# uw-math-ai/TheoremSearch

Hardware: AMD Instinct MI355X
Metric: queries/sec, brute-force top-10 over N x 768 theorem embeddings (higher is better)
Workload: dtype bf16; 1 GPU; 10000000x768 bf16 corpus, batch-256 queries, top-10 (BASELINE.json configs[2]); rows=10000000, dim=768, batch=256, k=10, searches_in_flight=1, parallelism=corpus row-sharded x1

## Files before the change

theoremsearch_amd/csrc/kernels_mfma16.h:

```cpp
#pragma once
#include <type_traits>

#include "kernels_mfma16_ops.h"
#include "kernels_screen8_tile.h"
#include "mfma16_variants.h"

namespace ts {

constexpr int kMfma16PrivCap = 16;
constexpr int kMfma16StageCap = 192;
constexpr int kMfma16StageBytes = 4 * kMfma16StageCap * 16 + 16;
constexpr int kMfma16PaceBytes = 256;

__device__ __forceinline__ u64 mfma16_block_test(const f32x4& a0, const f32x4& a1, float thr, float& m) {
    u64 mask;
    asm volatile(
        "v_max3_f32 %0, %2, %3, %4\n\t"
        "v_max3_f32 %0, %0, %5, %6\n\t"
        "v_max3_f32 %0, %0, %7, %8\n\t"
        "v_max_f32 %0, %0, %9\n\t"
        "v_cmp_ge_f32 %1, %0, %10"
        : "=&v"(m), "=s"(mask)
        : "v"(a0[0]), "v"(a0[1]), "v"(a0[2]), "v"(a0[3]), "v"(a1[0]), "v"(a1[1]), "v"(a1[2]), "v"(a1[3]), "v"(thr));
    return mask;
// ... 146 lines not shown
    constexpr int kUnits = dims::kUnits, kUnitBytes = dims::kUnitBytes, kSlots = dims::kSlots, kPieces = dims::kPieces;
    constexpr int kUnitK = dims::kUnitK;
    constexpr int kPieceEvery = kUnitSteps / kPieces;
    static_assert(kUnitSteps % kPieces == 0 && kPieceEvery >= 1, "DMA pieces must spread evenly over the k-steps");
    static_assert(!KSPLIT || (kUnitSteps == 4 && kPieces == 4), "k-split: four k-steps and four DMA pieces per unit and wave");
    static_assert(NB >= 1 && NB * kSteps * 4 <= 384, "query fragments must fit the register file");
    static_assert(!F32 || NB <= 2, "the fp32 issue order is written for one or two query blocks per wave");
    static_assert(kUnits == 1 || kUnits == 2 || kUnits == 4 || kUnits == 8, "units per tile");
    constexpr bool kStaged = !SPARSE;
    constexpr int kFrags = NB * kSteps;
    constexpr int kA = (kUnitSteps % 3 == 0) ? 3 : 4;
    constexpr int kQVmax = (KSPLIT || kLate) ? 24 : 36 - 2 * (kA - 2);
    constexpr int kQV = kFrags < kQVmax ? kFrags : kQVmax;
    constexpr bool kStreamNT = !PAIR;
    extern __shared__ __attribute__((aligned(16))) unsigned char smem[];
    const int lane = threadIdx.x & 63;
    const int wave = __builtin_amdgcn_readfirstlane(threadIdx.x >> 6);
    const int r16 = lane & 15, kq = lane >> 4;
    const int wg = PAIR ? (int)(((blockIdx.x >> 4) << 3) | (blockIdx.x & 7)) : (int)blockIdx.x;
    const int qhalf = PAIR ? (int)((blockIdx.x >> 3) & 1) : 0;
    const int G = PAIR ? (int)(gridDim.x >> 1) : (int)gridDim.x;
    const int nwriters = 4 * gridDim.x;
    const int writer = 4 * blockIdx.x + kq;
    const int khalf = KSPLIT ? (wave >> 1) : 0;
    int qid[NB];
#pragma unroll
    for (int b = 0; b < NB; ++b)
        qid[b] = KSPLIT ? qhalf * 128 + (((b + 2 * khalf) & 3) * 2 + (wave & 1)) * 16 + r16 : qhalf * 64 * NB + (b * 4 + wave) * 16 + r16;

    mfma_level_begin(a);
    uint4* stage = (uint4*)(smem + dims::kLds) + wave * kMfma16StageCap;
    uint2* stage8 = (uint2*)(smem + dims::kLds) + wave * kScreenStageCap;
    static_assert(kScreenStageCap * 8 == kMfma16StageCap * 16, "the screen's entries fill the same LDS");
    u32* stage_cnt = (u32*)(smem + dims::kLds + 4 * kMfma16StageCap * 16) + wave;
    if (kStaged && !I8 && lane == 0) *stage_cnt = 0;
    uint4* const xbuf = (uint4*)(smem + dims::kLds + kMfma16StageBytes + kMfma16PaceBytes);
    frag16 got[4] = {};
    const bool pace = PAIR && a.pair_pos != nullptr && a.pair_lag > 0 && wave == 0;
    unsigned* const pace_mine = PAIR ? a.pair_pos + 2 * wg + qhalf : nullptr;
    const unsigned* const pace_partner = PAIR ? a.pair_pos + 2 * wg + (1 - qhalf) : nullptr;
    unsigned pace_seen = 0, pace_prev = 0, pace_v;
    if (PAIR && wave == 0) ((u32*)(smem + dims::kLds + kMfma16StageBytes))[lane] = 0;
    const unsigned long long wg_start = (!SPARSE && a.wg_ticks) ? __builtin_amdgcn_s_memrealtime() : 0ull;
    const int64_t t0 = (!SPARSE && a.part) ? a.part[wg] : (a.ntiles * (int64_t)wg) / G;
    const int nt = (int)(((!SPARSE && a.part) ? a.part[wg + 1] : (a.ntiles * (int64_t)(wg + 1)) / G) - t0);
    if (nt <= 0) {
        if (!SPARSE && a.wg_ticks && threadIdx.x == 0 && qhalf == 0) a.wg_ticks[wg] = 0;
        if (!kStaged) {
#pragma unroll
            for (int b = 0; b < NB; ++b) a.pcount[(int64_t)qid[b] * nwriters + writer] = 0;
        }
        return;
    }
    const int nu = kUnits * nt;
    const int drow = 8 * wave + (lane >> 3);
    const int dchunk = (lane & 7) ^ ((drow >> 1) & 7);
    const int64_t tile_bytes = (int64_t)kTileRows * Deq * 2;
    const int64_t run_jump = tile_bytes * ((int64_t)a.run * a.tile_stride - a.run + 1);
    const int64_t g0 = (t0 / a.run) * a.run * a.tile_stride + t0 % a.run;
    const unsigned char* tile_src = (const unsigned char*)a.corpus + (int64_t)drow * (Deq * 2) + dchunk * 16 + g0 * tile_bytes;
    int issue_run_pos = (int)(t0 % a.run);
    int issue_u = 0, issue_ui = 0, issue_slot = 0;
    const unsigned lds_base = (unsigned)(unsigned long long)(__attribute__((address_space(3))) unsigned char*)smem;
    const unsigned lds0 = lds_base + wave * 1024;
    const unsigned pace_word = __builtin_amdgcn_readfirstlane(lds_base + dims::kLds + kMfma16StageBytes);
    const unsigned xfetch = lds_base + dims::kLds + kMfma16StageBytes + kMfma16PaceBytes + (((wave ^ 2) * 256 + lane) << 4);

    const int lane_off = (r16 >> 3) * 1024 + (r16 & 7) * 128;
    const int sw = (r16 >> 1) & 7;
    int xo[2];
#pragma unroll
    for (int sp = 0; sp < 2; ++sp) xo[sp] = lane_off + (((4 * sp + kq) ^ sw) << 4);
    const unsigned koff = KSPLIT ? (unsigned)(khalf * (kUnitSteps / 2) * 4096) : 0u;

#define TS16_ISSUED()                                                                 \
    do {                                                                              \
        if (++issue_ui == kUnits) {                                                   \
            issue_ui = 0;                                                             \
            tile_src += (issue_run_pos + 1 == a.run) ? run_jump : tile_bytes;         \
            issue_run_pos = (issue_run_pos + 1 == a.run) ? 0 : issue_run_pos + 1;     \
        }                                                                             \
        ++issue_u;                                                                    \
        issue_slot = (issue_slot + 1 == kSlots) ? 0 : issue_slot + 1;                 \
    } while (0)

    const int ahead = (a.ahead >= 2 && a.ahead < kSlots) ? a.ahead : kSlots - 1;
    for (int i = 0; i < ahead && issue_u < nu && !kNoDma; ++i) {
        const unsigned char* src = tile_src + issue_ui * (kUnitK * 2);
#pragma unroll
        for (int j = 0; j < kPieces; ++j) lds_dma16<kStreamNT>(src + j * 128, lds0 + issue_slot * kUnitBytes + j * 4096);
        TS16_ISSUED();
    }
    bf16x8 qv[kQV], qa[kFrags > kQV ? kFrags - kQV : 1];
#pragma unroll
    for (int b = 0; b < NB; ++b) {
        const bf16x8* pq = F32 ? (const bf16x8*)((const float*)a.q + (int64_t)qid[b] * D + 4 * kq)
                               : (const bf16x8*)(a.q + (int64_t)qid[b] * D + 8 * kq);
        if (KSPLIT) pq += 4 * kUnitSteps * khalf;
#pragma unroll
        for (int ks = 0; ks < kSteps; ++ks) {
            const int f = b * kSteps + ks;
            const int kabs = KSPLIT ? (ks / kUnitSteps) * kUnitStepsAll + (ks % kUnitSteps) : ks;
            if (f < kQV) qv[f < kQV ? f : 0] = pq[4 * kabs];
            else qa[f >= kQV ? f - kQV : 0] = pq[4 * kabs];
        }
    }
    float thr[NB];
#pragma unroll
    for (int b = 0; b < NB; ++b) thr[b] = mfma_level_thr(a, qid[b]);
    float fq1[I8 ? NB : 1], fq2[I8 ? NB : 1], fq3[I8 ? NB : 1];
    if constexpr (I8) {
#pragma unroll
        for (int b = 0; b < NB; ++b) {
            const float4 m4 = a.scr_q[qid[b]];
            screen_fold_query(thr[b], m4.x, m4.y, m4.z, fq1[b], fq2[b], fq3[b]);
        }
    }
#pragma unroll
    for (int f = 0; f < kFrags; ++f) {
        if (f < kQV) asm volatile("" : "+v"(qv[f < kQV ? f : 0]));
        else asm volatile("" : "+a"(qa[f >= kQV ? f - kQV : 0]));
    }
#pragma unroll
    for (int b = 0; b < NB; ++b) asm volatile("" : "+v"(thr[b]));
    if constexpr (I8) {
#pragma unroll
        for (int b = 0; b < NB; ++b) asm volatile("" : "+v"(fq1[b]), "+v"(fq2[b]), "+v"(fq3[b]));
    }

    asm volatile("s_waitcnt vmcnt(0)" ::: "memory");
    __builtin_amdgcn_s_barrier();
    asm volatile("" ::: "memory");

    frag16 af[2 * kA] = {};
    {
        const unsigned p0 = lds_base + xo[0] + (KSPLIT ? khalf * (kUnitSteps / 2) * 4096 : 0);
        const unsigned p1 = lds_base + xo[1] + (KSPLIT ? khalf * (kUnitSteps / 2) * 4096 : 0);
        lds_read16<0>(af[0], p0);
        lds_read16<2048>(af[1], p0);
        lds_read16<0>(af[2], p1);
        lds_read16<2048>(af[3], p1);
        if constexpr (kA > 3) {
            lds_read16<4096>(af[4], p0);
            lds_read16<4096 + 2048>(af[5], p0);
        }
        static_assert(kA == 3 || kA == 4, "prologue written for rings of 3 or 4 k-steps");
    }
    lds_ring_landed(af);

    f32x4 acc[2][NB];
    f32x4 accK[2][2][2] = {};
    f32x4 accL[kLate ? 2 : 1][2][kLate ? NB : 1];
    int lthr[kLate ? 2 : 1][kLate ? NB : 1];
    int lbest = 0;
    u64 lhit[kLate ? NB : 1];
    u64 lany = 0, lany2 = 0;
    if constexpr (kLate) {
#pragma unroll
        for (int b = 0; b < NB; ++b) {
            accL[1][0][b] = f32x4{0.0f, 0.0f, 0.0f, 0.0f};
            accL[1][1][b] = f32x4{0.0f, 0.0f, 0.0f, 0.0f};
            lthr[1][b] = 0x7fffffff;
            asm volatile("" : "+v"(accL[1][0][b]), "+v"(accL[1][1][b]), "+v"(lthr[1][b]));
        }
    }
    u32 cnt[NB];
#pragma unroll
    for (int b = 0; b < NB; ++b) cnt[b] = 0;
    int slot = 0, u = 0;
    unsigned long long t_vm = 0, t_bar = 0, t_dma = 0, t_all0 = 0;
    unsigned long long t_tail = 0;
    if (kStamps) t_all0 = cycle_stamp();
    unsigned long long c_begin = 0, r_begin = 0;
    if (kProbe) {
        c_begin = __builtin_amdgcn_s_memtime();
        r_begin = __builtin_amdgcn_s_memrealtime();
        __builtin_amdgcn_s_waitcnt(0xC07F);
    }

#define TS16_ACC(RB_, B_) (*((KSPLIT && (B_) < 2) ? &accK[par_][RB_][(B_) & 1] : &acc[RB_][B_]))
#define TS16_MMA(RB_, B_, KS_, AF_)                                                                        \
    do {                                                                                                   \
        constexpr int f_ = (B_) * kSteps + (KS_);                                                          \
        if constexpr (kLate) {                                                                             \
            if constexpr ((KS_) == 0 && f_ < kQV) mfma8_v_first(accL[par_][RB_][B_], AF_, qv[f_ < kQV ? f_ : 0]);  \
            else if constexpr ((KS_) == 0) mfma8_a_first(accL[par_][RB_][B_], AF_, qa[f_ >= kQV ? f_ - kQV : 0]); \
            else if constexpr (f_ < kQV) mfma8_v(accL[par_][RB_][B_], AF_, qv[f_ < kQV ? f_ : 0]);         \
            else mfma8_a(accL[par_][RB_][B_], AF_, qa[f_ >= kQV ? f_ - kQV : 0]);                          \
        } else if constexpr (I8) {                                                                         \
            if constexpr ((KS_) == 0 && f_ < kQV) mfma8_v_first(acc[RB_][B_], AF_, qv[f_ < kQV ? f_ : 0]);  \
            else if constexpr ((KS_) == 0) mfma8_a_first(acc[RB_][B_], AF_, qa[f_ >= kQV ? f_ - kQV : 0]); \
            else if constexpr (f_ < kQV) mfma8_v(acc[RB_][B_], AF_, qv[f_ < kQV ? f_ : 0]);                \
            else mfma8_a(acc[RB_][B_], AF_, qa[f_ >= kQV ? f_ - kQV : 0]);                                 \
        } else if constexpr ((KS_) == 0) {                                                                 \
            if constexpr (f_ < kQV) mfma16_v_first(TS16_ACC(RB_, B_), AF_, qv[f_ < kQV ? f_ : 0]);         \
            else mfma16_a_first(TS16_ACC(RB_, B_), AF_, qa[f_ >= kQV ? f_ - kQV : 0]);                     \
        } else {                                                                                           \
            if constexpr (f_ < kQV) mfma16_v(TS16_ACC(RB_, B_), AF_, qv[f_ < kQV ? f_ : 0]);               \
            else mfma16_a(TS16_ACC(RB_, B_), AF_, qa[f_ >= kQV ? f_ - kQV : 0]);                           \
        }                                                                                                  \
    } while (0)
#define TS16_MMAF(RB_, B_, KS_, AF_, I_)                                                                   \
    do {                                                                                                   \
        constexpr int f_ = (B_) * kSteps + (KS_);                                                          \
        const f32x4& af4_ = reinterpret_cast<const f32x4&>(AF_);                                           \
        if constexpr ((KS_) == 0 && (I_) == 0) {                                                           \
            if constexpr (f_ < kQV) mfma16f_v_first(acc[RB_][B_], af4_[I_], reinterpret_cast<const f32x4&>(qv[f_ < kQV ? f_ : 0])[I_]); \
            else mfma16f_a_first(acc[RB_][B_], af4_[I_], reinterpret_cast<const f32x4&>(qa[f_ >= kQV ? f_ - kQV : 0])[I_]); \
        } else if constexpr (f_ < kQV) {                                                                   \
            mfma16f_v(acc[RB_][B_], af4_[I_], reinterpret_cast<const f32x4&>(qv[f_ < kQV ? f_ : 0])[I_]);  \
        } else {                                                                                           \
            mfma16f_a(acc[RB_][B_], af4_[I_], reinterpret_cast<const f32x4&>(qa[f_ >= kQV ? f_ - kQV : 0])[I_]); \
        }                                                                                                  \
    } while (0)

#define TS16_LOAD(RB_, N_)                                                                                 \
    do {                                                                                                   \
        constexpr int w_ = 2 * ((N_) % kA) + (RB_);                                                        \
        if constexpr ((N_) < kUnitSteps) lds_read16<((N_) >> 1) * 4096 + (RB_) * 2048>(af[w_], ua[(N_) & 1]); \
        else lds_read16<(((N_) - kUnitSteps) >> 1) * 4096 + (RB_) * 2048>(af[w_], na[(N_) & 1]);          \
    } while (0)
#define TS16_PIECE(S_)                                                                                     \
    do {                                                                                                   \
        if constexpr ((S_) % kPieceEvery == kPieceEvery - 1)                                               \
            if (do_issue) {                                                                                \
                constexpr int j_ = (S_) / kPieceEvery;                                                     \
                unsigned long long d0_ = 0;                                                                \
                if (VARIANT == kVariantStamps) d0_ = cycle_stamp();                                        \
                if constexpr (steady_) lds_dma16s<j_ * 128, kStreamNT>(dma_voff, ssrc, idst + j_ * (4096 - 128 * TS16_DMA_IMM_LDS)); \
                else lds_dma16<kStreamNT>(isrc + j_ * 128, idst + j_ * 4096);                                         \
                if (VARIANT == kVariantStamps) t_dma += cycle_stamp() - d0_;                               \
            }                                                                                              \
    } while (0)
#define TS16_FILL(KS_, G_)                                                                                 \
    do {                                                                                                   \
        constexpr int fi_ = ((KS_) - (kSteps - 3)) * 4 + (G_);                                             \
        if constexpr (KSPLIT && !kNoEpi && (KS_) >= kSteps - 3) {                                          \
            if constexpr (fi_ == 0) {                                                                      \
                asm volatile("" : "+v"(got[0]), "+v"(got[1]), "+v"(got[2]), "+v"(got[3]));                 \
                ksplit_add4(sum_[0][0], accK[par_ ^ 1][0][0], reinterpret_cast<const f32x4&>(got[0]));               \
            }                                                                                              \
            if constexpr (fi_ == 1) ksplit_add4(sum_[1][0], accK[par_ ^ 1][1][0], reinterpret_cast<const f32x4&>(got[2])); \
            if constexpr (fi_ == 2) ksplit_add4(sum_[0][1], accK[par_ ^ 1][0][1], reinterpret_cast<const f32x4&>(got[1])); \
            if constexpr (fi_ == 3) ksplit_add4(sum_[1][1], accK[par_ ^ 1][1][1], reinterpret_cast<const f32x4&>(got[3])); \
            if constexpr (fi_ == 4) ksplit_test_a(best_[0], sum_[0][0], sum_[1][0]);                       \
            if constexpr (fi_ == 5) ksplit_test_b(best_[0], sum_[1][0]);                                   \
            if constexpr (fi_ == 6) ksplit_test_c(hit_[0], best_[0], thr[0]);                              \
            if constexpr (fi_ == 7) ksplit_test_a(best_[1], sum_[0][1], sum_[1][1]);                       \
            if constexpr (fi_ == 8) ksplit_test_b(best_[1], sum_[1][1]);                                   \
            if constexpr (fi_ == 9) ksplit_test_c(hit_[1], best_[1], thr[1]);                              \
        }                                                                                                  \
    } while (0)
#define TS16_THR8(KS_, G_)                                                                                 \
    do {                                                                                                   \
        if constexpr (I8 && !kNoEpi) {                                                                     \
            constexpr int gpk_ = NB >= 3 ? 4 : 2;                                                          \
            constexpr int g_ = NB == 1 ? (G_) + 2 : (G_);                                                  \
            constexpr int P_ = ((KS_) / 2) * gpk_ + g_;                                                    \
            if constexpr ((KS_) % 2 == 0 && g_ >= 0 && g_ < gpk_ && (NB == 1) == ((G_) < 0) && P_ < 4 * NB) { \
                if constexpr (kLate) screen_thr_piece<P_ & 3>(lthr[par_][P_ >> 2], tml[par_], fq1[P_ >> 2], fq2[P_ >> 2], fq3[P_ >> 2]); \
                else screen_thr_piece<P_ & 3>(ithr[P_ >> 2], tmc, fq1[P_ >> 2], fq2[P_ >> 2], fq3[P_ >> 2]);   \
            }                                                                                              \
        }                                                                                                  \
    } while (0)
#define TS16_LATE(KS_, G_)                                                                                 \
    do {                                                                                                   \
        if constexpr (kLate) {                                                                             \
            constexpr int p_ = (KS_) * 2 + (G_);                                                           \
            if constexpr (p_ < 3 * NB) {                                                                   \
                constexpr int b_ = p_ / 3;                                                                 \
                if constexpr (p_ % 3 == 0) late_test_a(lbest, accL[par_ ^ 1][0][b_], accL[par_ ^ 1][1][b_]); \
                if constexpr (p_ % 3 == 1) late_test_b(lbest, accL[par_ ^ 1][1][b_]);                      \
                if constexpr (p_ % 3 == 2) late_test_c(lhit[b_], lbest, lthr[par_ ^ 1][b_]);               \
            }                                                                                              \
            if constexpr (p_ == 3 * NB) late_or(lany, lhit[0], lhit[1]);                                   \
            if constexpr (p_ == 3 * NB + 1) late_or(lany2, lhit[2], lhit[3]);                              \
            if constexpr (p_ == 3 * NB + 2) late_or(lany, lany, lany2);                                    \
            if constexpr (steady_ && p_ == 2 * (kSteps - kA)) {    \
                asm volatile("" : "+s"(noff_l));                   \
                la_l[0] = lds_base + noff_l + xo[0] + koff;                                                \
                la_l[1] = lds_base + noff_l + xo[1] + koff;                                                \
                asm volatile("" : "+v"(la_l[0]), "+v"(la_l[1]));                                           \
                na[0] = la_l[0]; na[1] = la_l[1];                                                          \
            }                                                                                              \
            if constexpr (steady_ && p_ == 2 * kSteps - 2) {                                               \
                poff = soff;                                                                               \
                soff = noff_l;                                                                             \
                noff_l = (soff + kUnitBytes == (unsigned)dims::kLds) ? 0u : soff + kUnitBytes;             \
                s_tile += steady_jump;                                                                     \
                asm volatile("" : "+s"(poff), "+s"(soff), "+s"(noff_l), "+s"(s_tile));                     \
            }                                                                                              \
            if constexpr (steady_ && p_ == 2 * kSteps - 1) {                                               \
                sp_l += 1;                                                                                 \
                asm volatile("" : "+s"(sp_l));                                                             \
            }                                                                                              \
        }                                                                                                  \
    } while (0)
#ifndef TS16_ORDER_A
#define TS16_BF16_ORDER(KS_, R0_, N_, S_)                                                                  \
    do {                                                                                                   \
        if constexpr (KSPLIT) {                                                                            \
            TS16_MMA(0, 2, KS_, af[R0_]); TS16_LOAD(0, N_);                                                \
            TS16_MMA(1, 2, KS_, af[R0_ + 1]); TS16_LOAD(1, N_);                                            \
            TS16_MMA(0, 3, KS_, af[R0_]); TS16_MMA(1, 3, KS_, af[R0_ + 1]);                                \
            TS16_PIECE(S_);                                                                                \
            TS16_MMA(0, 0, KS_, af[R0_]); TS16_FILL(KS_, 0);                                               \
            TS16_MMA(1, 0, KS_, af[R0_ + 1]); TS16_FILL(KS_, 1);                                           \
            TS16_MMA(0, 1, KS_, af[R0_]); TS16_FILL(KS_, 2);                                               \
            TS16_MMA(1, 1, KS_, af[R0_ + 1]); TS16_FILL(KS_, 3);                                           \
            break;                                                                                         \
        }                                                                                                  \
        TS16_MMA(0, 0, KS_, af[R0_]); TS16_LOAD(0, N_); TS16_THR8(KS_, -2);                                \
        TS16_MMA(1, 0, KS_, af[R0_ + 1]); TS16_LOAD(1, N_); TS16_THR8(KS_, -1);                            \
        if constexpr (NB > 1) {                                                                            \
            TS16_MMA(0, 1, KS_, af[R0_]); TS16_THR8(KS_, 0);                                               \
            TS16_MMA(1, 1, KS_, af[R0_ + 1]); TS16_THR8(KS_, 1);                                           \
        }                                                                                                  \
        TS16_PIECE(S_);                                                                                    \
        if constexpr (NB > 2) {                                                                            \
            TS16_MMA(0, 2, KS_, af[R0_]); TS16_THR8(KS_, 2);                                               \
            TS16_MMA(1, 2, KS_, af[R0_ + 1]); TS16_THR8(KS_, 3);                                           \
        }                                                                                                  \
        if constexpr (NB > 3) { TS16_MMA(0, 3, KS_, af[R0_]); TS16_LATE(KS_, 0); TS16_MMA(1, 3, KS_, af[R0_ + 1]); TS16_LATE(KS_, 1); } \
    } while (0)
#else
#define TS16_BF16_ORDER(KS_, R0_, N_, S_)                                                                  \
    do {                                                                                                   \
        TS16_MMA(0, 0, KS_, af[R0_]); TS16_LOAD(0, N_);                                                    \
        if constexpr (NB > 1) { TS16_MMA(0, 1, KS_, af[R0_]); }                                            \
        TS16_LOAD(1, N_);                                                                                  \
        if constexpr (NB > 2) { TS16_MMA(0, 2, KS_, af[R0_]); }                                            \
        if constexpr (NB > 3) { TS16_MMA(0, 3, KS_, af[R0_]); }                                            \
        TS16_PIECE(S_);                                                                                    \
        TS16_MMA(1, 0, KS_, af[R0_ + 1]);                                                                  \
        if constexpr (NB > 1) { TS16_MMA(1, 1, KS_, af[R0_ + 1]); }                                        \
        if constexpr (NB > 2) { TS16_MMA(1, 2, KS_, af[R0_ + 1]); }                                        \
        if constexpr (NB > 3) { TS16_MMA(1, 3, KS_, af[R0_ + 1]); }                                        \
    } while (0)
#endif
#define TS16_STEP(UI, S_)                                                                                  \
    do {                                                                                                   \
        constexpr int ks_ = (UI) * kUnitSteps + (S_);                                                      \
        constexpr int r0_ = 2 * ((S_) % kA);                                                               \
        constexpr int n_ = (S_) + kA - 1;                                                                  \
        if constexpr (!kNoMma) {                                                                           \
             \
                         \
            if constexpr (kA == 3) asm volatile("s_waitcnt lgkmcnt(2)" : "+v"(af[r0_]), "+v"(af[r0_ + 1])); \
            else asm volatile("s_waitcnt lgkmcnt(4)" : "+v"(af[r0_]), "+v"(af[r0_ + 1]));                  \
        }                                                                                                  \
        if constexpr (!kNoMma && F32) {                                                                    \
                           \
            TS16_MMAF(0, 0, ks_, af[r0_], 0); TS16_LOAD(0, n_);                                            \
            TS16_MMAF(1, 0, ks_, af[r0_ + 1], 0); TS16_LOAD(1, n_);                                        \
            if constexpr (NB > 1) { TS16_MMAF(0, 1, ks_, af[r0_], 0); TS16_MMAF(1, 1, ks_, af[r0_ + 1], 0); } \
            TS16_MMAF(0, 0, ks_, af[r0_], 1); TS16_MMAF(1, 0, ks_, af[r0_ + 1], 1);                        \
            TS16_PIECE(S_);                                                                                \
            if constexpr (NB > 1) { TS16_MMAF(0, 1, ks_, af[r0_], 1); TS16_MMAF(1, 1, ks_, af[r0_ + 1], 1); } \
            TS16_MMAF(0, 0, ks_, af[r0_], 2); TS16_MMAF(1, 0, ks_, af[r0_ + 1], 2);                        \
            if constexpr (NB > 1) { TS16_MMAF(0, 1, ks_, af[r0_], 2); TS16_MMAF(1, 1, ks_, af[r0_ + 1], 2); } \
            TS16_MMAF(0, 0, ks_, af[r0_], 3); TS16_MMAF(1, 0, ks_, af[r0_ + 1], 3);                        \
            if constexpr (NB > 1) { TS16_MMAF(0, 1, ks_, af[r0_], 3); TS16_MMAF(1, 1, ks_, af[r0_ + 1], 3); } \
        }                                                                                                  \
        if constexpr (!kNoMma && !F32) {                                                                   \
             \
            TS16_BF16_ORDER(ks_, r0_, n_, S_);                                                             \
        }                                                                                                  \
        if constexpr (kNoMma) TS16_PIECE(S_);                                                              \
    } while (0)

#define TS16_KSPLIT_FETCH()                                                                                \
    do {                                                                                                   \
        lds_read16<0>(got[0], xfetch); lds_read16<1024>(got[1], xfetch);                                   \
        lds_read16<2048>(got[2], xfetch); lds_read16<3072>(got[3], xfetch);                                \
    } while (0)
#define TS16_UNIT_S(UI)                                                                                    \
    do {                                                                                                   \
        constexpr int cui_ = ((UI) + kSlots - 1) % kUnits;                                                 \
         \
        const unsigned noff = kLate ? noff_l : (soff + kUnitBytes == (unsigned)dims::kLds) ? 0u : soff + kUnitBytes; \
        unsigned ua[2], na[2];                                                                             \
        if constexpr (!kLate) {                                                                            \
            ua[0] = lds_base + soff + xo[0] + koff; ua[1] = lds_base + soff + xo[1] + koff;                \
            na[0] = lds_base + noff + xo[0] + koff; na[1] = lds_base + noff + xo[1] + koff;                \
        } else {    \
            ua[0] = la_l[0]; ua[1] = la_l[1];                                                              \
        }                                                                                                  \
        if constexpr (!kNoDma) wait_vmcnt<(kSlots - 3) * kPieces>();          \
        if constexpr (PAIR && (UI) == (2 % kUnits)) {                    \
             \
                            \
            asm volatile("v_readfirstlane_b32 %0, %1" : "=s"(pace_seen) : "v"(pace_v));                   \
            const int ahead_ = (int)((unsigned)t - pace_seen);                                             \
            if (pace && pace_seen != pace_prev && ahead_ > a.pair_lag && ahead_ < (1 << 20))               \
                for (int z_ = 0; z_ < ahead_ - a.pair_lag && z_ < 4; ++z_) __builtin_amdgcn_s_sleep(5);    \
            pace_prev = pace_seen;                                                                         \
        }                                                                                                  \
        __builtin_amdgcn_s_barrier();                                               \
        asm volatile("" ::: "memory");                                                                     \
        if constexpr (KSPLIT && (UI) == 2) TS16_KSPLIT_FETCH();                                            \
        if constexpr (PAIR && (UI) == 0) {                                                                 \
            if (pace) pair_publish_and_fetch(pace_mine, pace_partner, (unsigned)t, pace_word);            \
        }                                                                                                  \
        if constexpr (PAIR && (UI) == (1 % kUnits)) pair_read_word(pace_v, pace_word);                     \
        if (VARIANT == kVariantSleep) __builtin_amdgcn_s_sleep(4);                                         \
        constexpr bool do_issue = !kNoDma;                                                                 \
        constexpr bool steady_ = true;                                                                     \
        const unsigned char* isrc = nullptr;                                                               \
        const unsigned char* ssrc = s_tile + cui_ * (kUnitK * 2);                  \
        const unsigned idst = lds0 + poff;                                                                 \
        TS16_STEP(UI, 0); TS16_STEP(UI, 1); TS16_STEP(UI, 2); TS16_STEP(UI, 3);                            \
        if constexpr (kUnitSteps > 4) { TS16_STEP(UI, 4 % kUnitSteps); TS16_STEP(UI, 5 % kUnitSteps); TS16_STEP(UI, 6 % kUnitSteps); TS16_STEP(UI, 7 % kUnitSteps); } \
        if constexpr (kUnitSteps > 8) { TS16_STEP(UI, 8 % kUnitSteps); TS16_STEP(UI, 9 % kUnitSteps); TS16_STEP(UI, 10 % kUnitSteps); TS16_STEP(UI, 11 % kUnitSteps); } \
        if constexpr (!kLate) {                                                                            \
            if constexpr (cui_ == kUnits - 1 && !kNoDma) s_tile += steady_jump;                            \
            poff = soff;                                                                                   \
            soff = noff;                                                                                   \
        }                                                                                                  \
    } while (0)

#define TS16_UNIT(UI)                                                                                      \
    do {                                                                                                   \
        const int nslot = (slot + 1 == kSlots) ? 0 : slot + 1;                                             \
        unsigned ua[2], na[2];                                                                             \
        ua[0] = lds_base + slot * kUnitBytes + xo[0] + koff; ua[1] = lds_base + slot * kUnitBytes + xo[1] + koff;   \
        na[0] = lds_base + nslot * kUnitBytes + xo[0] + koff; na[1] = lds_base + nslot * kUnitBytes + xo[1] + koff; \
         \
        unsigned long long s0_ = 0, s1_ = 0;                                                               \
        if (kStamps) s0_ = cycle_stamp();                                                                  \
        if (u + 1 < nu && !kNoDma) wait_keep_units<kPieces>(issue_u - (u + 2));                            \
        if (kStamps) s1_ = cycle_stamp();                                                                  \
        __builtin_amdgcn_s_barrier();                                                                      \
        asm volatile("" ::: "memory");                                                                     \
        if constexpr (KSPLIT && (UI) == 2) TS16_KSPLIT_FETCH();                                            \
        if (kStamps) { t_vm += s1_ - s0_; t_bar += cycle_stamp() - s1_; }                                  \
        if (VARIANT == kVariantSleep) __builtin_amdgcn_s_sleep(4);    \
        const bool do_issue = issue_u < nu && !kNoDma;                                                     \
        constexpr bool steady_ = false;                                                                    \
        const unsigned char* isrc = tile_src + issue_ui * (kUnitK * 2);                                    \
        const unsigned char* ssrc = nullptr;                                                               \
         \
        const unsigned idst = __builtin_amdgcn_readfirstlane(lds0 + issue_slot * kUnitBytes);              \
        TS16_STEP(UI, 0); TS16_STEP(UI, 1); TS16_STEP(UI, 2); TS16_STEP(UI, 3);                            \
        if constexpr (kUnitSteps > 4) { TS16_STEP(UI, 4 % kUnitSteps); TS16_STEP(UI, 5 % kUnitSteps); TS16_STEP(UI, 6 % kUnitSteps); TS16_STEP(UI, 7 % kUnitSteps); } \
        if constexpr (kUnitSteps > 8) { TS16_STEP(UI, 8 % kUnitSteps); TS16_STEP(UI, 9 % kUnitSteps); TS16_STEP(UI, 10 % kUnitSteps); TS16_STEP(UI, 11 % kUnitSteps); } \
        if (do_issue) TS16_ISSUED();                                                                       \
        slot = nslot;                                                                                      \
        ++u;                                                                                               \
    } while (0)

#define TS16_KSPLIT_APPEND(TP)                                                                             \
    do {                                                                                                   \
        if (__builtin_expect((hit_[0] | hit_[1]) != 0, 0)) {                                               \
            const int64_t lt_ = t0 + (TP);                                                                 \
            const int64_t tile_row_ = (a.run == 1 ? lt_ * a.tile_stride : (lt_ / a.run) * a.run * a.tile_stride + lt_ % a.run) * kTileRows; \
            const int64_t row_base_ = tile_row_ + 4 * kq;                                                  \
            _Pragma("unroll") for (int i_ = 0; i_ < 2; ++i_)                                               \
                if (hit_[i_] != 0)                                                                         \
                    mfma16_append_block<kStaged>(sum_[0][i_], sum_[1][i_], thr[i_], best_[i_], qid[i_], writer, nwriters, cnt[i_], \
                                                 row_base_, a, stage, stage_cnt);                          \
        }                                                                                                  \
    } while (0)
    static_assert(kUnitSteps == 8 || kUnitSteps == 12 || (KSPLIT && kUnitSteps == 4), "unit = 8 or 12 k-steps of 32 (k-split: this wave's 4 of 8)");
    static_assert(kSlots >= 3, "the steady part keeps kSlots - 3 units in flight behind its wait");
    const int nt_steady = (a.run == 1 && ahead == kSlots - 1 && !kStamps && nu > ahead) ? (nu - ahead) / kUnits : 0;
    const int64_t steady_jump = tile_bytes * a.tile_stride;
    unsigned soff = 0, poff = (unsigned)(kSlots - 1) * kUnitBytes;
    unsigned noff_l = (unsigned)kUnitBytes;
    unsigned la_l[2] = {lds_base + xo[0] + koff, lds_base + xo[1] + koff};
    static_assert(!kLate || kUnits == 1, "the late-test screen advances the stream's tile base once per unit");
    const unsigned dma_voff = (unsigned)(drow * (Deq * 2) + dchunk * 16);
    const unsigned char* s_tile = (const unsigned char*)a.corpus + (t0 + ahead / kUnits) * steady_jump;
    f32x4 sum_[2][2] = {};
    float best_[2] = {};
    u64 hit_[2] = {};
    const tile_scalars_ptr scr_tile = (tile_scalars_ptr)a.scr_tile;
    f32x4 tmc = {0.0f, 0.0f, 0.0f, 0.0f}, tmn = {0.0f, 0.0f, 0.0f, 0.0f};
    f32x4 tml[2] = {{0.0f, 0.0f, 0.0f, 0.0f}, {0.0f, 0.0f, 0.0f, 0.0f}};
    tile_scalars_ptr sp_l = scr_tile + (t0 + 1);
    int ithr[I8 ? NB : 1];
    u32 scnt = 0, s_n = 0, s_nq = 0;
    int t_chk = 0;
    screen_u32_gptr s_count = nullptr;
    screen_u64_gptr s_cand = nullptr;
    screen_mask_cptr s_mask = nullptr;
    if constexpr (I8) {
        if constexpr (kLate) {
            screen_tile_scalars(tml[0], scr_tile, t0);
            screen_tile_scalars(tml[1], scr_tile, t0 + (nt > 1 ? 1 : 0));
            asm volatile("" : "+s"(tml[0]), "+s"(tml[1]), "+s"(sp_l));
        } else {
            screen_tile_scalars(tmc, scr_tile, t0);
            screen_tile_scalars(tmn, scr_tile, t0 + (nt > 1 ? 1 : 0));
            asm volatile("" : "+s"(tmc), "+s"(tmn));
        }
        const int64_t whole = a.n / kTileRows - t0;
        t_chk = whole < (int64_t)nt ? (whole > 0 ? (int)whole : 0) : nt;
        s_n = (u32)a.n;
        s_nq = (u32)a.nq_real;
        s_count = (screen_u32_gptr)a.count;
        s_cand = (screen_u64_gptr)a.cand;
        asm volatile("" : "+s"(scnt), "+s"(t_chk), "+s"(s_n), "+s"(s_nq), "+s"(s_count), "+s"(s_cand));
        if constexpr (kMasked8) {
            s_mask = (screen_mask_cptr)a.row_mask;
            asm volatile("" : "+s"(s_mask));
        }
    }
    constexpr int kTilePick = 0, kTileSteady = 1, kTileGeneral = 2;
    auto tile = [&](auto par_c, auto form_c, const int t) __attribute__((always_inline)) {
        constexpr int par_ = decltype(par_c)::value;
        constexpr int form_ = decltype(form_c)::value;
        (void)par_;
        unsigned long long tail0 = 0;
        if (form_ == kTileSteady || (form_ == kTilePick && t < nt_steady)) {
            TS16_UNIT_S(0);
            if constexpr (kUnits >= 2) TS16_UNIT_S(1 % kUnits);
            if constexpr (kUnits >= 4) {
                TS16_UNIT_S(2 % kUnits);
                TS16_UNIT_S(3 % kUnits);
            }
            if constexpr (kUnits == 8) {
                TS16_UNIT_S(4 % kUnits);
                TS16_UNIT_S(5 % kUnits);
                TS16_UNIT_S(6 % kUnits);
                TS16_UNIT_S(7 % kUnits);
            }
            if constexpr (!kNoMma) lds_ring_landed(af);
            if (form_ == kTilePick && t + 1 == nt_steady) {
                u = kUnits * nt_steady;
                slot = u % kSlots;
                issue_u = u + ahead;
                issue_ui = issue_u % kUnits;
                issue_slot = issue_u % kSlots;
                issue_run_pos = 0;
                tile_src = s_tile + dma_voff;
            }
        } else {
            TS16_UNIT(0);
            if constexpr (kUnits >= 2) TS16_UNIT(1 % kUnits);
            if constexpr (kUnits >= 4) {
                TS16_UNIT(2 % kUnits);
                TS16_UNIT(3 % kUnits);
            }
            if constexpr (kUnits == 8) {
                TS16_UNIT(4 % kUnits);
                TS16_UNIT(5 % kUnits);
                TS16_UNIT(6 % kUnits);
                TS16_UNIT(7 % kUnits);
            }
            if (VARIANT == kVariantScreenStamps) tail0 = cycle_stamp();
            if constexpr (!kNoMma) lds_ring_landed(af);
        }
        if constexpr (kNoMma) return;
        if constexpr (KSPLIT) {
            if constexpr (kNoEpi) {
                asm volatile("s_nop 15\n\ts_nop 3" : "+v"(accK[par_][0][0]), "+v"(accK[par_][0][1]), "+v"(accK[par_][1][0]), "+v"(accK[par_][1][1]),
                             "+v"(acc[0][2]), "+v"(acc[0][3]), "+v"(acc[1][2]), "+v"(acc[1][3]));
                return;
            }
            if (t > 0) TS16_KSPLIT_APPEND(t - 1);
            ksplit_hand_over(acc, xbuf + wave * 256 + lane);
            return;
        }
#ifdef TS16_ORDER_A
        mfma16_settle<NB>(acc);
#else
        if constexpr (NB < 4 || kNoEpi) mfma16_settle<NB>(acc);
#endif
        if constexpr (kNoEpi) {
#pragma unroll
            for (int b = 0; b < NB; ++b) asm volatile("" ::"v"(acc[0][b]), "v"(acc[1][b]));
            return;
        }
        if constexpr (kLate) {
            asm volatile("" : "+s"(tml[par_ ^ 1]));
            if constexpr (form_ == kTileSteady) tml[par_] = *(const volatile __attribute__((address_space(4))) f32x4*)sp_l;
            if (__builtin_expect(lany != 0, 0)) {
                const u32 tp = (u32)t0 + (u32)t - 1u;
                const u32 row_base = tp * kTileRows + 4 * kq;
                if (t - 1 >= t_chk) {
                    const u32 live = screen_tile_live<false>(tp * kTileRows, s_n, s_mask) >> (4 * kq);
#pragma unroll
                    for (int b = 0; b < NB; ++b)
                        if (lhit[b] != 0)
                            mfma8_append_block<true>(accL[par_ ^ 1][0][b], accL[par_ ^ 1][1][b], lthr[par_ ^ 1][b], qid[b], row_base, scnt, stage8, live, s_nq, s_count, s_cand);
                } else {
#pragma unroll
                    for (int b = 0; b < NB; ++b)
                        if (lhit[b] != 0)
                            mfma8_append_block<false>(accL[par_ ^ 1][0][b], accL[par_ ^ 1][1][b], lthr[par_ ^ 1][b], qid[b], row_base, scnt, stage8, 0u, s_nq, s_count, s_cand);
                }
            }
            if constexpr (form_ != kTileSteady) screen_tile_scalars(tml[par_], scr_tile, t0 + (t + 2 < nt ? t + 2 : nt - 1));
            return;
        }
        if constexpr (I8) {
            asm volatile("" : "+s"(tmn));
            u64 ihit[NB];
            const u64 iany = screen_tile_test<NB>(acc, ithr, ihit);
            if constexpr (variant_test_only(VARIANT)) {
                asm volatile("" ::"s"(iany));
            } else if (__builtin_expect(iany != 0, 0)) {
                const u32 row_base = ((u32)t0 + (u32)t) * kTileRows + 4 * kq;
                if (kMasked8 || t >= t_chk) {
                    const u32 live = screen_tile_live<kMasked8>(((u32)t0 + (u32)t) * kTileRows, s_n, s_mask) >> (4 * kq);
#pragma unroll
                    for (int b = 0; b < NB; ++b)
                        if (ihit[b] != 0)
                            mfma8_append_block<true>(acc[0][b], acc[1][b], ithr[b], qid[b], row_base, scnt, stage8, live, s_nq, s_count, s_cand);
                } else {
#pragma unroll
                    for (int b = 0; b < NB; ++b)
                        if (ihit[b] != 0)
                            mfma8_append_block<false>(acc[0][b], acc[1][b], ithr[b], qid[b], row_base, scnt, stage8, 0u, s_nq, s_count, s_cand);
                }
            }
            if (VARIANT == kVariantScreenStamps) t_tail += cycle_stamp() - tail0;
            tmc = tmn;
            screen_tile_scalars(tmn, scr_tile, t0 + (t + 2 < nt ? t + 2 : nt - 1));
            return;
        }
        mfma16_tile_tail<NB, VARIANT, kStaged>(acc, thr, qid, cnt, t0, t, kq, writer, nwriters, a, stage, stage_cnt);
    };
    using tile_pick = std::integral_constant<int, kTilePick>;
    if constexpr (kLate) {
        int t = 0;
        const int t_trips = __builtin_amdgcn_readfirstlane(nt_steady & ~1);
        if (t_trips > 0) {
            do {
                tile(std::integral_constant<int, 0>{}, std::integral_constant<int, kTileSteady>{}, t);
                tile(std::integral_constant<int, 1>{}, std::integral_constant<int, kTileSteady>{}, t + 1);
                t += 2;
            } while (t < t_trips);
        }
        if (t > 0) {
            u = kUnits * t;
            slot = u % kSlots;
            issue_u = u + ahead;
            issue_ui = issue_u % kUnits;
            issue_slot = issue_u % kSlots;
            issue_run_pos = 0;
            tile_src = s_tile + dma_voff;
        }
        asm volatile("s_waitcnt lgkmcnt(0)" : "+s"(tml[0]), "+s"(tml[1]));
        for (; t < nt; t += 2) {
            tile(std::integral_constant<int, 0>{}, std::integral_constant<int, kTileGeneral>{}, t);
            if (t + 1 >= nt) break;
            tile(std::integral_constant<int, 1>{}, std::integral_constant<int, kTileGeneral>{}, t + 1);
        }
    } else if constexpr (KSPLIT) {
        for (int t = 0; t < nt; t += 2) {
            tile(std::integral_constant<int, 0>{}, tile_pick{}, t);
            if (t + 1 < nt) tile(std::integral_constant<int, 1>{}, tile_pick{}, t + 1);
        }
    } else {
        for (int t = 0; t < nt; ++t) tile(std::integral_constant<int, 0>{}, tile_pick{}, t);
    }
    if constexpr (KSPLIT && !kNoEpi && !kNoMma) {
        asm volatile("s_waitcnt lgkmcnt(0)" ::: "memory");
        __builtin_amdgcn_s_barrier();
        asm volatile("" ::: "memory");
        TS16_KSPLIT_FETCH();
        asm volatile("s_waitcnt lgkmcnt(0)" : "+v"(got[0]), "+v"(got[1]), "+v"(got[2]), "+v"(got[3]));
        asm volatile("s_nop 15\n\ts_nop 3" : "+v"(accK[0][0][0]), "+v"(accK[0][0][1]), "+v"(accK[0][1][0]), "+v"(accK[0][1][1]),
                     "+v"(accK[1][0][0]), "+v"(accK[1][0][1]), "+v"(accK[1][1][0]), "+v"(accK[1][1][1]));
        f32x4 held[2][2];
#pragma unroll
        for (int rb = 0; rb < 2; ++rb)
#pragma unroll
            for (int i = 0; i < 2; ++i) held[rb][i] = ((nt - 1) & 1) ? accK[1][rb][i] : accK[0][rb][i];
#pragma unroll
        for (int rb = 0; rb < 2; ++rb)
#pragma unroll
            for (int i = 0; i < 2; ++i) sum_[rb][i] = held[rb][i] + reinterpret_cast<const f32x4&>(got[rb * 2 + i]);
        hit_[0] = mfma16_block_test(sum_[0][0], sum_[1][0], thr[0], best_[0]);
        hit_[1] = mfma16_block_test(sum_[0][1], sum_[1][1], thr[1], best_[1]);
        TS16_KSPLIT_APPEND(nt - 1);
    }
    if constexpr (kLate) {
        mfma16_settle<NB>(accL[0]);
        mfma16_settle<NB>(accL[1]);
        const bool odd = ((nt - 1) & 1) != 0;
        f32x4 fin[2][NB];
        int fthr[NB];
#pragma unroll
        for (int b = 0; b < NB; ++b) {
            fin[0][b] = odd ? accL[1][0][b] : accL[0][0][b];
            fin[1][b] = odd ? accL[1][1][b] : accL[0][1][b];
            fthr[b] = odd ? lthr[1][b] : lthr[0][b];
        }
        u64 fhit[NB];
        const u64 fany = screen_tile_test<NB>(fin, fthr, fhit);
        if (fany != 0) {
            const u32 tp = (u32)t0 + (u32)(nt - 1);
            const u32 row_base = tp * kTileRows + 4 * kq;
            if (nt - 1 >= t_chk) {
                const u32 live = screen_tile_live<false>(tp * kTileRows, s_n, s_mask) >> (4 * kq);
#pragma unroll
                for (int b = 0; b < NB; ++b)
                    if (fhit[b] != 0) mfma8_append_block<true>(fin[0][b], fin[1][b], fthr[b], qid[b], row_base, scnt, stage8, live, s_nq, s_count, s_cand);
            } else {
#pragma unroll
                for (int b = 0; b < NB; ++b)
                    if (fhit[b] != 0) mfma8_append_block<false>(fin[0][b], fin[1][b], fthr[b], qid[b], row_base, scnt, stage8, 0u, s_nq, s_count, s_cand);
            }
        }
    }
#undef TS16_LATE
#undef TS16_KSPLIT_APPEND
#undef TS16_KSPLIT_FETCH
#undef TS16_UNIT
#undef TS16_UNIT_S
#undef TS16_STEP
#undef TS16_MMA
#undef TS16_ACC
#undef TS16_MMAF
#undef TS16_LOAD
#undef TS16_BF16_ORDER
#undef TS16_FILL
#undef TS16_THR8
#undef TS16_PIECE
#undef TS16_ISSUED
    if (I8 && !variant_test_only(VARIANT)) {
        screen_flush_stage(stage8, scnt, lane, s_count, s_cand);
    } else if (kStaged && !I8) {
        mfma16_flush_stage(a, stage, stage_cnt, lane);
    } else {
#pragma unroll
        for (int b = 0; b < NB; ++b) a.pcount[(int64_t)qid[b] * nwriters + writer] = cnt[b];
    }
    if (!SPARSE && a.wg_ticks && threadIdx.x == 0 && qhalf == 0)
        a.wg_ticks[wg] = (unsigned)(__builtin_amdgcn_s_memrealtime() - wg_start);
    if (kStamps && a.dbg && lane == 0)
        mfma16_write_stamps(a.dbg + ((size_t)blockIdx.x * 4 + wave) * 4, t_all0, t_vm, t_bar, VARIANT == kVariantScreenStamps ? t_tail : t_dma);
    if (kProbe && a.dbg && threadIdx.x == 0) mfma16_write_probe(a.dbg, c_begin, r_begin, nu);
}

}
```

theoremsearch_amd/csrc/kernels_mfma16_ops.h:

```cpp
#pragma once
#include "kernels_mfma.h"

namespace ts {

typedef __attribute__((ext_vector_type(4))) float f32x4;
typedef __attribute__((ext_vector_type(4))) unsigned frag16;

__device__ __forceinline__ void mfma16_v_first(f32x4& acc, const frag16& a, const bf16x8& b) {
    asm volatile("v_mfma_f32_16x16x32_bf16 %0, %1, %2, 0" : "=&v"(acc) : "v"(a), "v"(b));
}
__device__ __forceinline__ void mfma16_v(f32x4& acc, const frag16& a, const bf16x8& b) {
    asm volatile("v_mfma_f32_16x16x32_bf16 %0, %1, %2, %0" : "+v"(acc) : "v"(a), "v"(b));
}
__device__ __forceinline__ void mfma16_a_first(f32x4& acc, const frag16& a, const bf16x8& b) {
    asm volatile("v_mfma_f32_16x16x32_bf16 %0, %1, %2, 0" : "=&v"(acc) : "v"(a), "a"(b));
}
__device__ __forceinline__ void mfma16_a(f32x4& acc, const frag16& a, const bf16x8& b) {
    asm volatile("v_mfma_f32_16x16x32_bf16 %0, %1, %2, %0" : "+v"(acc) : "v"(a), "a"(b));
}
__device__ __forceinline__ void mfma8_v_first(f32x4& acc, const frag16& a, const bf16x8& b) {
    asm volatile("v_mfma_i32_16x16x64_i8 %0, %1, %2, 0" : "=&v"(acc) : "v"(a), "v"(b));
}
__device__ __forceinline__ void mfma8_v(f32x4& acc, const frag16& a, const bf16x8& b) {
    asm volatile("v_mfma_i32_16x16x64_i8 %0, %1, %2, %0" : "+v"(acc) : "v"(a), "v"(b));
}
__device__ __forceinline__ void mfma8_a_first(f32x4& acc, const frag16& a, const bf16x8& b) {
    asm volatile("v_mfma_i32_16x16x64_i8 %0, %1, %2, 0" : "=&v"(acc) : "v"(a), "a"(b));
}
__device__ __forceinline__ void mfma8_a(f32x4& acc, const frag16& a, const bf16x8& b) {
    asm volatile("v_mfma_i32_16x16x64_i8 %0, %1, %2, %0" : "+v"(acc) : "v"(a), "a"(b));
}
__device__ __forceinline__ void mfma16f_v_first(f32x4& acc, float a, float b) {
    asm volatile("v_mfma_f32_16x16x4_f32 %0, %1, %2, 0" : "=&v"(acc) : "v"(a), "v"(b));
}
__device__ __forceinline__ void mfma16f_v(f32x4& acc, float a, float b) {
    asm volatile("v_mfma_f32_16x16x4_f32 %0, %1, %2, %0" : "+v"(acc) : "v"(a), "v"(b));
}
__device__ __forceinline__ void mfma16f_a(f32x4& acc, float a, float b) {
    asm volatile("v_mfma_f32_16x16x4_f32 %0, %1, %2, %0" : "+v"(acc) : "v"(a), "a"(b));
}
__device__ __forceinline__ void mfma16f_a_first(f32x4& acc, float a, float b) {
    asm volatile("v_mfma_f32_16x16x4_f32 %0, %1, %2, 0" : "=&v"(acc) : "v"(a), "a"(b));
}
template <int OFF>
__device__ __forceinline__ void lds_read16(frag16& dst, unsigned addr) {
    static_assert(OFF >= 0 && OFF < 65536, "ds_read offset field");
    asm volatile("ds_read_b128 %0, %1 offset:%2" : "=v"(dst) : "v"(addr), "n"(OFF));
}
#ifndef TS16_DMA_IMM_LDS
#define TS16_DMA_IMM_LDS 1
#endif
template <int IMM, bool NT = true>
__device__ __forceinline__ void lds_dma16s(unsigned voff, const void* sbase, unsigned lds_dst) {
    static_assert(IMM >= 0 && IMM < 4096, "13-bit signed immediate");
    if constexpr (NT)
        asm volatile(
            "s_mov_b32 m0, %2\n\t"
            "s_nop 0\n\t"
            "global_load_lds_dwordx4 %0, %1 offset:%3" TS_DMA_POLICY
            :
            : "v"(voff), "s"(sbase), "s"(lds_dst), "n"(IMM)
            : "memory");
    else
        asm volatile(
            "s_mov_b32 m0, %2\n\t"
            "s_nop 0\n\t"
            "global_load_lds_dwordx4 %0, %1 offset:%3"
            :
            : "v"(voff), "s"(sbase), "s"(lds_dst), "n"(IMM)
            : "memory");
}
template <int N>
__device__ __forceinline__ void lds_ring_landed(frag16 (&af)[N]) {
    static_assert(N == 6 || N == 8, "ring of 3 or 4 k-steps, two row blocks");
    if constexpr (N == 6)
        asm volatile("s_waitcnt lgkmcnt(0)" : "+v"(af[0]), "+v"(af[1]), "+v"(af[2]), "+v"(af[3]), "+v"(af[4]), "+v"(af[5]));
    else
        asm volatile("s_waitcnt lgkmcnt(0)" : "+v"(af[0]), "+v"(af[1]), "+v"(af[2]), "+v"(af[3]), "+v"(af[4]), "+v"(af[5]),
                     "+v"(af[6]), "+v"(af[7]));
}
template <int NB>
__device__ __forceinline__ void mfma16_settle(f32x4 (&acc)[2][NB]) {
    if constexpr (NB == 4)
        asm volatile("s_nop 15\n\ts_nop 3" : "+v"(acc[0][0]), "+v"(acc[0][1]), "+v"(acc[0][2]), "+v"(acc[0][3]), "+v"(acc[1][0]),
                     "+v"(acc[1][1]), "+v"(acc[1][2]), "+v"(acc[1][3]));
    else if constexpr (NB == 3)
        asm volatile("s_nop 15\n\ts_nop 3" : "+v"(acc[0][0]), "+v"(acc[0][1]), "+v"(acc[0][2]), "+v"(acc[1][0]), "+v"(acc[1][1]),
                     "+v"(acc[1][2]));
    else if constexpr (NB == 2)
        asm volatile("s_nop 15\n\ts_nop 3" : "+v"(acc[0][0]), "+v"(acc[0][1]), "+v"(acc[1][0]), "+v"(acc[1][1]));
    else
        asm volatile("s_nop 15\n\ts_nop 3" : "+v"(acc[0][0]), "+v"(acc[1][0]));
}

}
```

Measured before the change: 158,400 queries/s.

## Reschedule late-test screen and split M0 setup from LDS DMA issue

```diff
diff --git a/theoremsearch_amd/csrc/kernels_mfma16.h b/theoremsearch_amd/csrc/kernels_mfma16.h
--- a/theoremsearch_amd/csrc/kernels_mfma16.h
+++ b/theoremsearch_amd/csrc/kernels_mfma16.h
@@ -322,7 +322,7 @@
     f32x4 accK[2][2][2] = {};
     f32x4 accL[kLate ? 2 : 1][2][kLate ? NB : 1];
     int lthr[kLate ? 2 : 1][kLate ? NB : 1];
-    int lbest = 0;
+    int lbest[2] = {0, 0};
     u64 lhit[kLate ? NB : 1];
     u64 lany = 0, lany2 = 0;
     if constexpr (kLate) {
@@ -397,10 +397,16 @@
                 constexpr int j_ = (S_) / kPieceEvery;                                                     \
                 unsigned long long d0_ = 0;                                                                \
                 if (VARIANT == kVariantStamps) d0_ = cycle_stamp();                                        \
-                if constexpr (steady_) lds_dma16s<j_ * 128, kStreamNT>(dma_voff, ssrc, idst + j_ * (4096 - 128 * TS16_DMA_IMM_LDS)); \
+                if constexpr (steady_ && kLate) lds_dma16s_go<j_ * 128, kStreamNT>(dma_voff, ssrc);        \
+                else if constexpr (steady_) lds_dma16s<j_ * 128, kStreamNT>(dma_voff, ssrc, idst + j_ * (4096 - 128 * TS16_DMA_IMM_LDS)); \
                 else lds_dma16<kStreamNT>(isrc + j_ * 128, idst + j_ * 4096);                                         \
                 if (VARIANT == kVariantStamps) t_dma += cycle_stamp() - d0_;                               \
             }                                                                                              \
+    } while (0)
+#define TS16_PIECE_M0(S_)                                                                                  \
+    do {                                                                                                   \
+        if constexpr (kLate && steady_ && !kNoDma && (S_) % kPieceEvery == kPieceEvery - 1)                \
+            lds_dma16s_m0<((S_) / kPieceEvery) * (4096 - 128 * TS16_DMA_IMM_LDS)>(idst);                   \
     } while (0)
 #define TS16_FILL(KS_, G_)                                                                                 \
     do {                                                                                                   \
@@ -428,7 +434,9 @@
             constexpr int g_ = NB == 1 ? (G_) + 2 : (G_);                                                  \
             constexpr int P_ = ((KS_) / 2) * gpk_ + g_;                                                    \
             if constexpr ((KS_) % 2 == 0 && g_ >= 0 && g_ < gpk_ && (NB == 1) == ((G_) < 0) && P_ < 4 * NB) { \
-                if constexpr (kLate) screen_thr_piece<P_ & 3>(lthr[par_][P_ >> 2], tml[par_], fq1[P_ >> 2], fq2[P_ >> 2], fq3[P_ >> 2]); \
+                 \
+                 \
+                if constexpr (kLate) screen_thr_piece<(P_ >> 2)>(lthr[par_][P_ & 3], tml[par_], fq1[P_ & 3], fq2[P_ & 3], fq3[P_ & 3]); \
                 else screen_thr_piece<P_ & 3>(ithr[P_ >> 2], tmc, fq1[P_ >> 2], fq2[P_ >> 2], fq3[P_ >> 2]);   \
             }                                                                                              \
         }                                                                                                  \
@@ -436,33 +444,50 @@
 #define TS16_LATE(KS_, G_)                                                                                 \
     do {                                                                                                   \
         if constexpr (kLate) {                                                                             \
-            constexpr int p_ = (KS_) * 2 + (G_);                                                           \
-            if constexpr (p_ < 3 * NB) {                                                                   \
-                constexpr int b_ = p_ / 3;                                                                 \
-                if constexpr (p_ % 3 == 0) late_test_a(lbest, accL[par_ ^ 1][0][b_], accL[par_ ^ 1][1][b_]); \
-                if constexpr (p_ % 3 == 1) late_test_b(lbest, accL[par_ ^ 1][1][b_]);                      \
-                if constexpr (p_ % 3 == 2) late_test_c(lhit[b_], lbest, lthr[par_ ^ 1][b_]);               \
+            constexpr int at_ = (KS_) * 4 + (G_);                                                          \
+            constexpr int o_ = par_ ^ 1;                                                                   \
+             \
+            if constexpr (at_ == 0 * 4 + 0) late_test_a(lbest[0], accL[o_][0][0], accL[o_][1][0]);         \
+            if constexpr (at_ == 1 * 4 + 2) late_test_a(lbest[1], accL[o_][0][1], accL[o_][1][1]);         \
+            if constexpr (at_ == 1 * 4 + 0) late_test_b(lbest[0], accL[o_][1][0]);                         \
+            if constexpr (at_ == 2 * 4 + 0) late_test_b(lbest[1], accL[o_][1][1]);                         \
+            if constexpr (at_ == 2 * 4 + 1) late_test_c(lhit[0], lbest[0], lthr[o_][0]);                   \
+            if constexpr (at_ == 3 * 4 + 2) late_test_a(lbest[0], accL[o_][0][2], accL[o_][1][2]);         \
+            if constexpr (at_ == 3 * 4 + 3) late_test_c(lhit[1], lbest[1], lthr[o_][1]);                   \
+            if constexpr (at_ == 3 * 4 + 0) late_test_a(lbest[1], accL[o_][0][3], accL[o_][1][3]);         \
+            if constexpr (at_ == 4 * 4 + 0) late_test_b(lbest[0], accL[o_][1][2]);                         \
+            if constexpr (at_ == 5 * 4 + 2) late_test_b(lbest[1], accL[o_][1][3]);                         \
+            if constexpr (at_ == 5 * 4 + 3) late_test_c(lhit[2], lbest[0], lthr[o_][2]);                   \
+            if constexpr (at_ == 6 * 4 + 0) late_test_c(lhit[3], lbest[1], lthr[o_][3]);                   \
+            if constexpr (at_ == 6 * 4 + 1) late_or(lany, lhit[0], lhit[1]);                               \
+            if constexpr (at_ == 8 * 4 + 0) late_or(lany2, lhit[2], lhit[3]);                              \
+            if constexpr (at_ == 10 * 4 + 0) late_or(lany, lany, lany2);                                   \
+            if constexpr (steady_ && at_ == 0 * 4 + 1) {           \
+                asm volatile("" : "+s"(nring[par_]));                                                      \
+                idst = lds0 + nring[par_];                                                                 \
+                asm volatile("" : "+s"(idst));                                                             \
             }                                                                                              \
-            if constexpr (p_ == 3 * NB) late_or(lany, lhit[0], lhit[1]);                                   \
-            if constexpr (p_ == 3 * NB + 1) late_or(lany2, lhit[2], lhit[3]);                              \
-            if constexpr (p_ == 3 * NB + 2) late_or(lany, lany, lany2);                                    \
-            if constexpr (steady_ && p_ == 2 * (kSteps - kA)) {    \
-                asm volatile("" : "+s"(noff_l));                   \
-                la_l[0] = lds_base + noff_l + xo[0] + koff;                                                \
-                la_l[1] = lds_base + noff_l + xo[1] + koff;                                                \
+            if constexpr (steady_ && at_ == 4 * (kSteps - kA - 1) + 2) {    \
+                asm volatile("" : "+s"(nring[o_]));                                                        \
+                nring[par_] = (nring[o_] + kUnitBytes == (unsigned)dims::kLds) ? 0u : nring[o_] + kUnitBytes; \
+                asm volatile("" : "+s"(nring[par_]));                                                      \
+            }                                                                                              \
+            if constexpr (steady_ && at_ == 4 * (kSteps - kA) + 0) {    \
+                asm volatile("" : "+s"(nring[par_]));              \
+                la_l[0] = lds_base + nring[par_] + xo[0] + koff;                                           \
+                la_l[1] = lds_base + nring[par_] + xo[1] + koff;                                           \
                 asm volatile("" : "+v"(la_l[0]), "+v"(la_l[1]));                                           \
                 na[0] = la_l[0]; na[1] = la_l[1];                                                          \
             }                                                                                              \
-            if constexpr (steady_ && p_ == 2 * kSteps - 2) {                                               \
-                poff = soff;                                                                               \
-                soff = noff_l;                                                                             \
-                noff_l = (soff + kUnitBytes == (unsigned)dims::kLds) ? 0u : soff + kUnitBytes;             \
-                s_tile += steady_jump;                                                                     \
-                asm volatile("" : "+s"(poff), "+s"(soff), "+s"(noff_l), "+s"(s_tile));                     \
-            }                                                                                              \
-            if constexpr (steady_ && p_ == 2 * kSteps - 1) {                                               \
+            if constexpr (steady_ && at_ == 4 * (kSteps - 2) + 2) {                                        \
+                asm volatile("" : "+s"(sp_l));                                                             \
                 sp_l += 1;                                                                                 \
                 asm volatile("" : "+s"(sp_l));                                                             \
+            }                                                                                              \
+            if constexpr (steady_ && at_ == 4 * (kSteps - 1) + 2) {    \
+                asm volatile("" : "+s"(s_tile));                                                           \
+                s_tile += steady_jump;                                                                     \
+                asm volatile("" : "+s"(s_tile));                                                           \
             }                                                                                              \
         }                                                                                                  \
     } while (0)
@@ -483,13 +508,13 @@
         TS16_MMA(0, 0, KS_, af[R0_]); TS16_LOAD(0, N_); TS16_THR8(KS_, -2);                                \
         TS16_MMA(1, 0, KS_, af[R0_ + 1]); TS16_LOAD(1, N_); TS16_THR8(KS_, -1);                            \
         if constexpr (NB > 1) {                                                                            \
-            TS16_MMA(0, 1, KS_, af[R0_]); TS16_THR8(KS_, 0);                                               \
+            TS16_MMA(0, 1, KS_, af[R0_]); TS16_THR8(KS_, 0); TS16_PIECE_M0(S_);                            \
             TS16_MMA(1, 1, KS_, af[R0_ + 1]); TS16_THR8(KS_, 1);                                           \
         }                                                                                                  \
         TS16_PIECE(S_);                                                                                    \
         if constexpr (NB > 2) {                                                                            \
-            TS16_MMA(0, 2, KS_, af[R0_]); TS16_THR8(KS_, 2);                                               \
-            TS16_MMA(1, 2, KS_, af[R0_ + 1]); TS16_THR8(KS_, 3);                                           \
+            TS16_MMA(0, 2, KS_, af[R0_]); TS16_THR8(KS_, 2); TS16_LATE(KS_, 2);                            \
+            TS16_MMA(1, 2, KS_, af[R0_ + 1]); TS16_THR8(KS_, 3); TS16_LATE(KS_, 3);                        \
         }                                                                                                  \
         if constexpr (NB > 3) { TS16_MMA(0, 3, KS_, af[R0_]); TS16_LATE(KS_, 0); TS16_MMA(1, 3, KS_, af[R0_ + 1]); TS16_LATE(KS_, 1); } \
     } while (0)
@@ -516,7 +541,14 @@
         if constexpr (!kNoMma) {                                                                           \
              \
                          \
-            if constexpr (kA == 3) asm volatile("s_waitcnt lgkmcnt(2)" : "+v"(af[r0_]), "+v"(af[r0_ + 1])); \
+             \
+             \
+             \
+            if constexpr (kLate && steady_) {                                                              \
+                static_assert(!kLate || kA == 3, "lgkmcnt(2)");                                            \
+                asm volatile("" : "+v"(af[r0_]), "+v"(af[r0_ + 1]));                                       \
+                __builtin_amdgcn_s_waitcnt(0xC27F);                              \
+            } else if constexpr (kA == 3) asm volatile("s_waitcnt lgkmcnt(2)" : "+v"(af[r0_]), "+v"(af[r0_ + 1])); \
             else asm volatile("s_waitcnt lgkmcnt(4)" : "+v"(af[r0_]), "+v"(af[r0_ + 1]));                  \
         }                                                                                                  \
         if constexpr (!kNoMma && F32) {                                                                    \
@@ -548,7 +580,7 @@
     do {                                                                                                   \
         constexpr int cui_ = ((UI) + kSlots - 1) % kUnits;                                                 \
          \
-        const unsigned noff = kLate ? noff_l : (soff + kUnitBytes == (unsigned)dims::kLds) ? 0u : soff + kUnitBytes; \
+        const unsigned noff = kLate ? 0u : (soff + kUnitBytes == (unsigned)dims::kLds) ? 0u : soff + kUnitBytes; \
         unsigned ua[2], na[2];                                                                             \
         if constexpr (!kLate) {                                                                            \
             ua[0] = lds_base + soff + xo[0] + koff; ua[1] = lds_base + soff + xo[1] + koff;                \
@@ -578,7 +610,7 @@
         constexpr bool steady_ = true;                                                                     \
         const unsigned char* isrc = nullptr;                                                               \
         const unsigned char* ssrc = s_tile + cui_ * (kUnitK * 2);                  \
-        const unsigned idst = lds0 + poff;                                                                 \
+        unsigned idst = lds0 + poff;                  \
         TS16_STEP(UI, 0); TS16_STEP(UI, 1); TS16_STEP(UI, 2); TS16_STEP(UI, 3);                            \
         if constexpr (kUnitSteps > 4) { TS16_STEP(UI, 4 % kUnitSteps); TS16_STEP(UI, 5 % kUnitSteps); TS16_STEP(UI, 6 % kUnitSteps); TS16_STEP(UI, 7 % kUnitSteps); } \
         if constexpr (kUnitSteps > 8) { TS16_STEP(UI, 8 % kUnitSteps); TS16_STEP(UI, 9 % kUnitSteps); TS16_STEP(UI, 10 % kUnitSteps); TS16_STEP(UI, 11 % kUnitSteps); } \
@@ -610,7 +642,7 @@
         const unsigned char* isrc = tile_src + issue_ui * (kUnitK * 2);                                    \
         const unsigned char* ssrc = nullptr;                                                               \
          \
-        const unsigned idst = __builtin_amdgcn_readfirstlane(lds0 + issue_slot * kUnitBytes);              \
+        unsigned idst = __builtin_amdgcn_readfirstlane(lds0 + issue_slot * kUnitBytes);                    \
         TS16_STEP(UI, 0); TS16_STEP(UI, 1); TS16_STEP(UI, 2); TS16_STEP(UI, 3);                            \
         if constexpr (kUnitSteps > 4) { TS16_STEP(UI, 4 % kUnitSteps); TS16_STEP(UI, 5 % kUnitSteps); TS16_STEP(UI, 6 % kUnitSteps); TS16_STEP(UI, 7 % kUnitSteps); } \
         if constexpr (kUnitSteps > 8) { TS16_STEP(UI, 8 % kUnitSteps); TS16_STEP(UI, 9 % kUnitSteps); TS16_STEP(UI, 10 % kUnitSteps); TS16_STEP(UI, 11 % kUnitSteps); } \
@@ -636,7 +668,7 @@
     const int nt_steady = (a.run == 1 && ahead == kSlots - 1 && !kStamps && nu > ahead) ? (nu - ahead) / kUnits : 0;
     const int64_t steady_jump = tile_bytes * a.tile_stride;
     unsigned soff = 0, poff = (unsigned)(kSlots - 1) * kUnitBytes;
-    unsigned noff_l = (unsigned)kUnitBytes;
+    unsigned nring[2] = {(unsigned)(kSlots - 1) * kUnitBytes, 0u};
     unsigned la_l[2] = {lds_base + xo[0] + koff, lds_base + xo[1] + koff};
     static_assert(!kLate || kUnits == 1, "the late-test screen advances the stream's tile base once per unit");
     const unsigned dma_voff = (unsigned)(drow * (Deq * 2) + dchunk * 16);
@@ -890,6 +922,7 @@
 #undef TS16_FILL
 #undef TS16_THR8
 #undef TS16_PIECE
+#undef TS16_PIECE_M0
 #undef TS16_ISSUED
     if (I8 && !variant_test_only(VARIANT)) {
         screen_flush_stage(stage8, scnt, lane, s_count, s_cand);
diff --git a/theoremsearch_amd/csrc/kernels_mfma16_ops.h b/theoremsearch_amd/csrc/kernels_mfma16_ops.h
--- a/theoremsearch_amd/csrc/kernels_mfma16_ops.h
+++ b/theoremsearch_amd/csrc/kernels_mfma16_ops.h
@@ -70,6 +70,17 @@
             : "v"(voff), "s"(sbase), "s"(lds_dst), "n"(IMM)
             : "memory");
 }
+template <int OFF>
+__device__ __forceinline__ void lds_dma16s_m0(unsigned lds_dst) {
+    if constexpr (OFF == 0) asm volatile("s_mov_b32 m0, %0" : : "s"(lds_dst));
+    else asm volatile("s_add_i32 m0, %0, %1" : : "s"(lds_dst), "n"(OFF) : "scc");
+}
+template <int IMM, bool NT = true>
+__device__ __forceinline__ void lds_dma16s_go(unsigned voff, const void* sbase) {
+    static_assert(IMM >= 0 && IMM < 4096, "13-bit signed immediate");
+    if constexpr (NT) asm volatile("global_load_lds_dwordx4 %0, %1 offset:%2" TS_DMA_POLICY : : "v"(voff), "s"(sbase), "n"(IMM) : "memory");
+    else asm volatile("global_load_lds_dwordx4 %0, %1 offset:%2" : : "v"(voff), "s"(sbase), "n"(IMM) : "memory");
+}
 template <int N>
 __device__ __forceinline__ void lds_ring_landed(frag16 (&af)[N]) {
     static_assert(N == 6 || N == 8, "ring of 3 or 4 k-steps, two row blocks");
```

After: 160,500 queries/s, median of 6. 1.3% higher.
